# ARPA-SIMC/CRITERIA3D

Measured on AMD Instinct MI355X. Metric: simulated-hours/sec on 512x512x20 grid, higher is better.
Workload: dtype f64

## Files before the change

### criteria3d_amd/csrc/sf3d_control.inc

```

#define SYS_STORE(p, x) __hip_atomic_store((p), (x), __ATOMIC_RELAXED, __HIP_MEMORY_SCOPE_SYSTEM)
#define SYS_LOAD(p) __hip_atomic_load((p), __ATOMIC_RELAXED, __HIP_MEMORY_SCOPE_SYSTEM)

__device__ __forceinline__ unsigned long long rec_lo(double x, uint32_t tag) { return ((unsigned long long)__double_as_longlong(x) & 0xFFFFFFFFull) | ((unsigned long long)tag << 32); }
__device__ __forceinline__ unsigned long long rec_hi(double x, uint32_t tag) { return ((unsigned long long)__double_as_longlong(x) >> 32) | ((unsigned long long)tag << 32); }
__device__ __forceinline__ bool rec_ok(unsigned long long a, unsigned long long b, uint32_t tag) { return (uint32_t)(a >> 32) == tag && (uint32_t)(b >> 32) == tag; }
__device__ __forceinline__ double rec_value(unsigned long long a, unsigned long long b) { return __longlong_as_double((long long)((a & 0xFFFFFFFFull) | (b << 32))); }

__device__ __forceinline__ void dist_combine(double (&acc)[4], const double (&x)[4], int K, int op, bool first)
{
    if (first) { for (int k = 0; k < K; ++k) acc[k] = x[k]; return; }
    if (op == 1) { for (int k = 0; k < K; ++k) acc[k] = dmax(acc[k], x[k]); return; }
    if (op >= 2) {
        dd_merge(acc[0], acc[1], x[0], x[1]);
        if (op == 3) dd_merge(acc[2], acc[3], x[2], x[3]); else for (int k = 2; k < K; ++k) acc[k] += x[k];
        return;
    }
    for (int k = 0; k < K; ++k) acc[k] += x[k];
}
template <int K>
__device__ __forceinline__ bool dist_allgather(const DevView& v, Ctrl* c, double (&vals)[K], int op)
{
    static_assert(K >= 1 && K <= 4, "a mailbox holds four values");
    if (v.world <= 1) return true;
// ... 233 lines not shown
__device__ __forceinline__ void dist_put_node(const DevView& v, uint32_t i, uint32_t par, int field, double val)
{
    const DistView* d = v.dist;
    const uint32_t q = i >> 6, lane = i & 63u;
    for (uint32_t t = d->bndStart[q], t1 = d->bndStart[q + 1]; t < t1; ++t)
        if (d->bndLane[t] == lane) {
            const uint32_t p = d->bndPeer[t];
            SYS_STORE(d->payload[p] + d->sendOff[p] + (size_t)(par * SF3D_DIST_FIELDS + field) * d->sendCount[p] + d->bndSlot[t], val);
        }
}


__device__ __forceinline__ void begin_attempt(Ctrl* c)
{
    c->dt = dmin(c->dtCurr, c->maxTimeStep);
    c->hold = c->cur;
    c->best = -1;
    c->bestMBR = NODATA_D;
    c->approx = 0;
    c->counters[0]++;
    c->stage = ST_APPROX;
}

__global__ void k_step_begin(Ctrl* c, double maxTimeStep)
{
    c->maxTimeStep = maxTimeStep;
    c->seqCount = 0;
    c->aBuf ^= 1u;
    begin_attempt(c);
}

__device__ __forceinline__ void reject_attempt(Ctrl* c)
{
    c->seSource = 2;
    c->cur = c->hold;
    begin_attempt(c);
}

#ifndef SF3D_PROBE_BUDGET
#define SF3D_PROBE_BUDGET 8u
#endif
__device__ __forceinline__ void courant_decision(Ctrl* c, double cmax)
{
    c->counters[2]++;
    c->courant = cmax;
    c->asmSeq++; c->asmSurfOnly = (cmax < 1.01 || c->dt <= c->dtMin) ? 0u : 1u;
    if (cmax < 1.01 || c->dt <= c->dtMin) {
        uint32_t budget = (uint32_t)((c->approx + 1) * ((float)c->maxIter / (float)c->maxApprox));
        c->iterBudget = budget > 25u ? budget : 25u;
        c->iter = 0;
        c->bestNorm = 1.;
// ... 164 lines not shown
```

### criteria3d_amd/csrc/sf3d_device.h

```cpp
#ifndef SF3D_DEVICE_H
#define SF3D_DEVICE_H

#include <stdint.h>

#define SF3D_SLOTS 10
#define SF3D_POOL 5
#define SF3D_BLOCK 256
#define SF3D_CHUNK 64
#define SF3D_MAX_BLOCKS 2048
#define CK_NONE 0
#define CK_MIXED 255

enum : uint8_t { LK_NONE = 0, LK_SOIL_VERT = 1, LK_SOIL_LAT = 2, LK_RUNOFF = 3, LK_INFILTRATION = 4 };

enum : uint32_t {
    ST_IDLE = 0,
    ST_ATTEMPT = 1,
    ST_APPROX = 2,
    ST_SWEEP = 3,
    ST_POST = 4,
    ST_RESTORE = 5,
    ST_ACCEPT = 6,
    ST_DONE = 7,
    ST_FAIL = 8
};

struct alignas(16) sf3d_d2 { double x, y; };
struct alignas(8) sf3d_f2 { float x, y; };

struct SoilDev {
// ... 201 lines not shown
    uint32_t nbSurf, nbSoil;
    double probeMin;
    const uint32_t* chunkList; uint32_t nList, nListSurf;
    const uint32_t* asmList;
    uint32_t pLo, pHi;
    uint32_t aLo, aHi;
    const uint32_t* bndList; uint32_t nBnd;
    const uint16_t* lmask;
    uint32_t haloDirect;
    uint32_t ntStream;
    const DistView* dist;
    int32_t world, rank;
    const uint8_t* owner;
    const ChunkDesc* cdesc;
    const double *z, *size, *pond, *sink;
    const uint16_t* cls;
    const uint8_t* btype;
    const double *bslope, *bsize, *prescribed;
    const uint32_t* lto;
    const uint8_t* lkind;
    const uint8_t* probeMask;
    const double *larea, *ldist;
    double* lflowSum;
    sf3d_d2* A2x[2];
    double *b, *C;
    double* X[SF3D_POOL];
    double *Se, *SeHold, *K, *flow, *bflowRate, *bflowSum;
    double* compatCv; uint8_t* compatCn; double* compatDiag;
    double *cgDiag, *cgR, *cgP, *cgQ;
    double *part0, *part1;
    double *part2, *part3;
    unsigned int* arrive;
    unsigned int* gridBar;
    const SoilDev* soils;
    const double* roughness;
    PairGrid pair;
    ResGrid res;
    Ctrl* ctrl;
    HeatDev heat;
};

struct MapGeo {
    double cohesion;
    double tanFriction;
    double bulkDensity;
    double present;
};
// ... 119 lines not shown
```

### criteria3d_amd/csrc/sf3d_host_build.inc

```

namespace {

template <class F> void parallel_for(uint32_t n, F f)
{
    unsigned nt = std::thread::hardware_concurrency();
    if (nt == 0) nt = 1;
    if (nt > 16) nt = 16;
    if (n < 65536 || nt == 1) { f(0u, n); return; }
    std::vector<std::thread> th;
    const uint32_t chunk = (n + nt - 1) / nt;
    for (unsigned t = 0; t < nt; ++t) {
        const uint32_t a = t * chunk, b = (a + chunk < n) ? a + chunk : n;
        if (a >= b) break;
        th.emplace_back([=] { f(a, b); });
    }
    for (auto& t : th) t.join();
}

const char* kKernelNames[KID_COUNT] = {"k_props", "k_assemble", "k_sweep", "k_post", "k_restore", "k_accept", "k_sweep_pair", "k_sweep_resident", "k_output_map"};

}

sf3d_error_t sf3d_partition_bounds(uint32_t ns, int world, uint32_t* bounds)
{
// ... 92 lines not shown
    }
};

struct SnowCache { float* base = nullptr; uint8_t* mine = nullptr; uint32_t nCells = 0; double lastMs = 0.; bool hourDone = false; };
struct CropCache { float* base = nullptr; CropUnitDev* units = nullptr; uint8_t* mine = nullptr; uint32_t nCells = 0, nUnits = 0; double lastMs[2] = {0., 0.}; };

struct RootCache {
    char* cells = nullptr;
    char* tables = nullptr;
    double* out = nullptr;
    uint8_t* mine = nullptr;
    size_t off[16] = {0};
    uint32_t nCells = 0, nUnits = 0, nSoils = 0, nRows = 0, nrLayers = 0, lunetteMax = 0;
    bool computed = false;
    double lastMs[3] = {0., 0., 0.};
};

struct DeviceSolver::Impl {
    int device = -1;
    hipStream_t stream = nullptr;
    hipStream_t stream2 = nullptr;
    hipEvent_t evLinks[2] = {nullptr, nullptr};
    bool linksPending[2] = {false, false};
    int overlapAccept = -1;
    DevView v{};
    Ctrl* hostCtrl = nullptr;
    std::vector<void*> allocs;
    uint32_t N = 0, ns = 0;
    uint32_t ownedNodes = 0;
    uint32_t lastSweeps = 8;
    uint32_t lastBatches = 1;
    uint32_t predCount = 0, pred[16] = {0};
    uint32_t lastHeatSweeps = 8;
    std::vector<uint32_t> gsLevelStart;
    uint32_t lastHeatSteps = 1;
    double* heatOut[6] = {nullptr};
    double* heatAirP = nullptr;
    std::vector<std::pair<uint32_t, hipGraphExec_t>> graphs;
    int useFused = -1;
    int useGraphs = -1;
    Partition part;
    DistWindow* window = nullptr;
    size_t windowBytes = 0;
    std::vector<void*> peerMaps;
    DistView hostDist{};
    DistView* devDist = nullptr;
// ... 87 lines not shown
             fatal_ = true;                                                                    \
             return SF3D_SOLVER_ERROR; } } while (0)

DeviceSolver& DeviceSolver::instance() { static DeviceSolver s; return s; }
const char* DeviceSolver::kernel_name(int kid) { return (kid >= 0 && kid < KID_COUNT) ? kKernelNames[kid] : nullptr; }

sf3d_error_t DeviceSolver::set_device(int dev)
{
    if (!impl_) impl_ = new Impl();
    int count = 0;
    HIP_TRY(hipGetDeviceCount(&count));
    if (dev < 0 || dev >= count) { snprintf(err_, sizeof(err_), "device %d out of range (%d visible)", dev, count); return SF3D_SOLVER_ERROR; }
    impl_->device = dev;
    HIP_TRY(hipSetDevice(dev));
    return SF3D_OK;
}

static uint64_t g_deviceBytes = 0;
sf3d_error_t DeviceSolver::release()
{
    if (!impl_) return SF3D_OK;
    Impl& I = *impl_;
    if (I.stream) hipStreamSynchronize(I.stream);
    if (I.stream2) hipStreamSynchronize(I.stream2);
    if (I.stream3) hipStreamSynchronize(I.stream3);
#if SF3D_RES_PROFILE
    if (built_ && I.v.res.on && I.v.res.pub) {
        double pr[32];
        if (hipMemcpy(pr, I.v.res.pub, sizeof(pr), hipMemcpyDeviceToHost) == hipSuccess && pr[16] > 0.) {
            const char* names[7] = {"compute + record stores issued", "wave sum + block partial", "halo records", "partial records of all blocks", "barrier B", "norm + decision", "(prologue: per launch, not per iteration)"};
            fprintf(stderr, "[sf3d] resident sweep loop, block 0: %.0f launches, %.2f iterations per launch, %.2f us per launch\n", pr[16], pr[15] / pr[16], pr[17] / pr[16] / 100.);
            for (int p = 0; p < 7; ++p) fprintf(stderr, "[sf3d]   %-40s %7.2f us per iteration\n", names[p], pr[8 + p] / pr[15] / 100.);
        }
    }
#endif
    I.linksPending[0] = I.linksPending[1] = false;
    if (I.stream3) {
        (void)hipStreamDestroy(I.stream3); I.stream3 = nullptr;
        for (auto& ev : I.evSlab) if (ev) { (void)hipEventDestroy(ev); ev = nullptr; }
    }
    I.slabs = -1;
    for (auto& p : I.pending) { I.freeEvents.push_back(p.a); I.freeEvents.push_back(p.b); }
    I.pending.clear();
    for (auto& g : I.graphs) hipGraphExecDestroy(g.second);
    I.graphs.clear();
    for (void* p : I.allocs) hipFree(p);
    I.allocs.clear();
    g_deviceBytes = 0;
    I.maps.free_all();
    if (I.comm && I.pCommDestroy) { I.pCommDestroy(I.comm); I.comm = nullptr; }
    I.rcclMode = false; I.rcclMine = I.rcclGathered = nullptr;
    for (void* p : I.peerMaps) hipIpcCloseMemHandle(p);
    I.peerMaps.clear();
    I.drop_shm();
    if (I.window) { hipFree(I.window); I.window = nullptr; }
    I.devDist = nullptr; I.distStats = nullptr;
    connected_ = false;
    built_ = false;
    fatal_ = false;
    I.overlapAccept = I.useFused = I.useGraphs = I.residentGrids = -1;
    return SF3D_OK;
}

sf3d_error_t DeviceSolver::synchronize()
{
    if (!impl_ || !impl_->stream) return SF3D_OK;
    HIP_TRY(hipStreamSynchronize(impl_->stream));
    if (impl_->stream2) { HIP_TRY(hipStreamSynchronize(impl_->stream2)); impl_->linksPending[0] = impl_->linksPending[1] = false; }
    return SF3D_OK;
}

template <class T> static hipError_t dev_alloc(std::vector<void*>& allocs, T*& p, size_t count)
{
    void* q = nullptr;
    hipError_t e = hipMalloc(&q, (count ? count : 1) * sizeof(T));
    if (e == hipSuccess) { allocs.push_back(q); p = static_cast<T*>(q); g_deviceBytes += (uint64_t)(count ? count : 1) * sizeof(T); }
    return e;
}
uint64_t DeviceSolver::device_bytes() const { return g_deviceBytes; }

static void fill_params(Ctrl& c, const ParamsHost& p)
{
    c.MBRThreshold = p.MBRThreshold; c.residualTolerance = p.residualTolerance;
    c.dtMin = p.dtMin; c.dtMax = p.dtMax; c.lvRatio = p.lvRatio;
    c.courantThreshold = p.courantThreshold; c.instabilityFactor = p.instabilityFactor;
    c.maxApprox = p.maxApprox; c.maxIter = p.maxIter; c.wrc = p.wrc; c.meanType = p.meanType;
    c.dtCurr = p.dtCurr;
    c.lineal = p.lineal ? 1u : 0u;
}

sf3d_error_t DeviceSolver::ensure_device()
// ... 6 lines not shown
        int count = 0;
        HIP_TRY(hipGetDeviceCount(&count));
        if (count <= 0) { snprintf(err_, sizeof(err_), "no HIP device visible: the soilFluxes3D product path has no CPU fallback"); return SF3D_SOLVER_ERROR; }
        if (const char* de = getenv("SF3D_DEVICES")) {
            std::vector<int> list;
            for (const char* q = de; *q;) { char* end = nullptr; const long v = strtol(q, &end, 10); if (end == q) break; list.push_back((int)v); q = (*end == ',') ? end + 1 : end; }
            if (!list.empty()) {
                const int pick = list[(size_t)(dev < 0 ? 0 : dev) % list.size()];
                if (pick < 0 || pick >= count) { snprintf(err_, sizeof(err_), "SF3D_DEVICES names device %d, %d visible", pick, count); return SF3D_SOLVER_ERROR; }
                dev = pick;
            }
        }
        I.device = dev % count;
    }
    HIP_TRY(hipSetDevice(I.device));
    if (!I.stream) HIP_TRY(hipStreamCreateWithFlags(&I.stream, hipStreamNonBlocking));
    return SF3D_OK;
}

sf3d_error_t DeviceSolver::sync_to_device(HostModel& m, const ParamsHost& p)
{
    { const sf3d_error_t e = ensure_device(); if (e != SF3D_OK) return e; }
    Impl& I = *impl_;
    if ((I.linksPending[0] || I.linksPending[1]) && (m.graphDirty || m.stateDirty || m.flowSumsDirty || !built_)) { HIP_TRY(hipStreamSynchronize(I.stream2)); I.linksPending[0] = I.linksPending[1] = false; }
    if (!I.hostCtrl) HIP_TRY(hipHostMalloc((void**)&I.hostCtrl, sizeof(Ctrl), hipHostMallocDefault));

    const uint32_t N = m.N, ns = m.ns;
    const size_t NS = (size_t)N * SF3D_SLOTS;

    if (m.graphDirty || !built_) {
        if (world_ > 1 && connected_) { snprintf(err_, sizeof(err_), "topology changed after sf3d_dist_connect: call sf3d_dist_prepare / export / connect again"); return SF3D_TOPOGRAPHY_ERROR; }
        if (m.surf.size() < N || m.hasClass.size() < N) { snprintf(err_, sizeof(err_), "the model's build arrays were released (a trimmed strip): re-initialise before changing the topology"); return SF3D_TOPOGRAPHY_ERROR; }
        for (uint32_t i = 0; i < N; ++i) {
            if ((m.surf[i] != 0) != (i < ns)) { snprintf(err_, sizeof(err_), "node %u: surface nodes must be exactly the first nrSurfaceNodes indices", i); return SF3D_TOPOGRAPHY_ERROR; }
            if (!m.hasClass[i]) { snprintf(err_, sizeof(err_), "node %u has no soil/surface class", i); return SF3D_MISSING_DATA_ERROR; }
        }
        if (built_) { if (m.hostStaleState) fetch_state(m); if (m.hostStaleFlows) fetch_flows(m); if (m.heat && m.hostStaleHeat && I.v.heat.on) fetch_heat(m); }
        release();
        I.N = N; I.ns = ns;
        DevView& v = I.v;
        v = DevView{};
        v.N = N; v.ns = ns; v.Nnorm = m.globalN ? m.globalN : N;
        v.nChunks = (N + SF3D_CHUNK - 1) / SF3D_CHUNK;
        v.qSplit = (ns + SF3D_CHUNK - 1) / SF3D_CHUNK;
        if (v.qSplit > v.nChunks) v.qSplit = v.nChunks;

        std::vector<uint8_t> kind(NS, LK_NONE);
// ... 360 lines not shown
                            const size_t e = (size_t)sl * N + i;
                            if (kind[e] != LK_NONE && to[e] / SF3D_CHUNK > far) far = to[e] / SF3D_CHUNK;
                        }
                    I.propsNeed[q] = far + 1;
                }
            });
            for (uint32_t q = 1; q < nChunks; ++q) if (I.propsNeed[q] < I.propsNeed[q - 1]) I.propsNeed[q] = I.propsNeed[q - 1];
        }
        {
            const uint32_t per = SF3D_BLOCK / SF3D_CHUNK;
            auto blocks = [&](uint32_t chunks) { uint32_t b = (chunks + per - 1) / per; if (b > SF3D_MAX_BLOCKS) b = SF3D_MAX_BLOCKS; return b; };
            v.nbSoil = blocks(v.nList - v.nListSurf);
            if (const char* be = getenv("SF3D_ASM_SOIL_BLOCKS")) { const uint32_t nb = (uint32_t)atoi(be); if (nb > 0 && nb < v.nbSoil) v.nbSoil = nb; }
        }
        double *z, *size, *pond, *sink, *bslope, *bsize, *prescribed, *roughness, *larea, *ldist;
        uint16_t* cls; uint8_t *btype, *lkind; uint32_t* lto; SoilDev* soils; ChunkDesc* dcdesc;
        HIP_TRY(dev_alloc(I.allocs, z, N)); HIP_TRY(dev_alloc(I.allocs, size, N));
        HIP_TRY(dev_alloc(I.allocs, pond, N)); HIP_TRY(dev_alloc(I.allocs, sink, N));
        HIP_TRY(dev_alloc(I.allocs, cls, N)); HIP_TRY(dev_alloc(I.allocs, btype, N));
        HIP_TRY(dev_alloc(I.allocs, bslope, N)); HIP_TRY(dev_alloc(I.allocs, bsize, N));
        HIP_TRY(dev_alloc(I.allocs, prescribed, N));
        HIP_TRY(dev_alloc(I.allocs, lto, NS)); HIP_TRY(dev_alloc(I.allocs, lkind, NS));
        HIP_TRY(dev_alloc(I.allocs, larea, NS)); HIP_TRY(dev_alloc(I.allocs, ldist, NS));
        HIP_TRY(dev_alloc(I.allocs, v.lflowSum, NS)); HIP_TRY(dev_alloc(I.allocs, v.A2x[0], NS / 2)); HIP_TRY(dev_alloc(I.allocs, v.A2x[1], NS / 2));
        HIP_TRY(dev_alloc(I.allocs, v.b, N)); HIP_TRY(dev_alloc(I.allocs, v.C, N));
        for (int k = 0; k < SF3D_POOL; ++k) HIP_TRY(dev_alloc(I.allocs, v.X[k], N));
        HIP_TRY(dev_alloc(I.allocs, v.Se, N)); HIP_TRY(dev_alloc(I.allocs, v.K, N)); HIP_TRY(dev_alloc(I.allocs, v.SeHold, N));
        HIP_TRY(dev_alloc(I.allocs, dcdesc, (size_t)nChunks));
        uint32_t* dlist; HIP_TRY(dev_alloc(I.allocs, dlist, listSurf.size()));
        if (!listSurf.empty()) HIP_TRY(hipMemcpy(dlist, listSurf.data(), listSurf.size() * 4, hipMemcpyHostToDevice));
        v.chunkList = dlist;
        v.asmList = dlist;
        v.owner = nullptr; v.dist = nullptr;
        {
            const char* e = getenv("SF3D_NT_STREAM");
            const double sweepBytes = 152.0 * (double)v.nList * SF3D_CHUNK;
            v.ntStream = e ? (e[0] != '0') : (sweepBytes > 256.0 * 1024 * 1024);
        }
        {
            v.probeMin = 0.8;
            if (const char* ce = getenv("SF3D_COURANT_PROBE")) { v.probeMin = atof(ce); if (ce[0] == '0' && ce[1] == 0) v.probeMin = -1.; if (ce[0] == 'a') v.probeMin = 0.; }
        }
        I.pairBlocks = 0; I.pairMasked = false; v.pair.masked = 0;
        uint32_t pairOwnLo = 0, pairOwnHi = pairNY;
        if (!pairNode.empty() && world_ > 1) {
            bool ok = true;
            std::vector<int8_t> rowMine(pairNY, -1);
// ... 653 lines not shown
```

### criteria3d_amd/csrc/sf3d_host_step.inc

```
sf3d_error_t DeviceSolver::fetch_state(HostModel& m)
{
    Impl& I = *impl_;
    HIP_TRY(hipMemcpyAsync(m.H.data(), I.v.X[mirror_.cur], (size_t)m.N * 8, hipMemcpyDeviceToHost, I.stream));
    HIP_TRY(hipMemcpyAsync(m.Se.data(), I.v.Se, (size_t)m.N * 8, hipMemcpyDeviceToHost, I.stream));
    HIP_TRY(hipMemcpyAsync(m.K.data(), I.v.K, (size_t)m.N * 8, hipMemcpyDeviceToHost, I.stream));
    HIP_TRY(hipStreamSynchronize(I.stream));
    m.hostStaleState = false;
    return SF3D_OK;
}

sf3d_error_t DeviceSolver::fetch_flows(HostModel& m)
{
    Impl& I = *impl_;
    const size_t N = m.N;
    if (I.stream2) { HIP_TRY(hipStreamSynchronize(I.stream2)); I.linksPending[0] = I.linksPending[1] = false; }
    HIP_TRY(hipMemcpyAsync(m.bflowSum.data(), I.v.bflowSum, N * 8, hipMemcpyDeviceToHost, I.stream));
    HIP_TRY(hipMemcpyAsync(m.bflowRate.data(), I.v.bflowRate, N * 8, hipMemcpyDeviceToHost, I.stream));
    if (I.dslot.empty()) {
        for (int s = 0; s < SF3D_SLOTS; ++s)
            HIP_TRY(hipMemcpyAsync(m.lflowSum[s].data(), I.v.lflowSum + (size_t)s * N, N * 8, hipMemcpyDeviceToHost, I.stream));
        HIP_TRY(hipStreamSynchronize(I.stream));
    } else {
        I.stage.resize(N * SF3D_SLOTS);
        HIP_TRY(hipMemcpyAsync(I.stage.data(), I.v.lflowSum, N * SF3D_SLOTS * 8, hipMemcpyDeviceToHost, I.stream));
        HIP_TRY(hipStreamSynchronize(I.stream));
        for (int s = 0; s < SF3D_SLOTS; ++s) {
            const uint8_t* d = I.dslot.data() + (size_t)s * N; double* dst = m.lflowSum[s].data();
            for (size_t i = 0; i < N; ++i) dst[i] = I.stage[(size_t)d[i] * N + i];
        }
    }
    m.hostStaleFlows = false;
    return SF3D_OK;
}

sf3d_error_t DeviceSolver::fetch_heat(HostModel& m)
{
    Impl& I = *impl_;
    const size_t N = m.N;
// ... 647 lines not shown
            if (I.residentGrids == 0) nbk = SF3D_MAX_BLOCKS;
            I.residentBlocks.push_back({fn, nbk});
        }
        return dim3(v.nb < nbk ? v.nb : nbk);
    };
    if (heatOn && multi) I.useFused = 1;
    const bool fused = !multi && I.useFused;
    const bool fusedMulti = multi && I.useFused;
    const bool linealOn = p.lineal && v.cgDiag != nullptr && !multi && I.useFused;
    const bool resOn = v.res.on && I.resBlocks != 0 && (fused || (fusedMulti && v.haloDirect && !I.rcclMode)) && !linealOn;
    if (resOn && !multi) {
        static const long failAt = getenv("SF3D_RESIDENT_FAIL_TEST") ? strtol(getenv("SF3D_RESIDENT_FAIL_TEST"), nullptr, 10) : -1;
        I.v.res.forceTimeout = (failAt >= 0 && (long)I.stepSeqAll == failAt) ? 1u : 0u;
        ++I.stepSeqAll;
    }
    const bool pairOn = !resOn && (fused || (fusedMulti && v.haloDirect && v.nBnd != 0)) && I.pairBlocks != 0 && !linealOn;
    const dim3 pgrid(I.pushBlocks ? I.pushBlocks : 1);
    hipStream_t st = I.stream;

    const bool timedStep = I.timing == 1 || (I.timing == 2 && (I.stepSeq++ % 8 == 0));
    if (I.overlapAccept < 0) { const char* oe = getenv("SF3D_OVERLAP_ACCEPT"); I.overlapAccept = (oe && oe[0] == '0') ? 0 : 1; }
    if (I.overlapAccept && !multi && !I.stream2) { HIP_TRY(hipStreamCreateWithFlags(&I.stream2, hipStreamNonBlocking)); HIP_TRY(hipEventCreateWithFlags(&I.evLinks[0], hipEventDisableTiming)); HIP_TRY(hipEventCreateWithFlags(&I.evLinks[1], hipEventDisableTiming)); }
    const bool overlap = I.overlapAccept && !multi && I.stream2 && !timedStep && I.timing != 1 && v.compatCv == nullptr;
    auto timed = [&](int kid, auto launch) {
        if (!timedStep || (I.timing == 2 && kid != KID_SWEEP && kid != KID_SWEEP_PAIR && kid != KID_SWEEP_RES)) { launch(); return; }
        hipEvent_t a, b;
        if (I.freeEvents.size() >= 2) { a = I.freeEvents.back(); I.freeEvents.pop_back(); b = I.freeEvents.back(); I.freeEvents.pop_back(); }
        else { hipEventCreate(&a); hipEventCreate(&b); }
        hipEventRecord(a, st); launch(); hipEventRecord(b, st);
        I.pending.push_back({a, b, kid});
    };

    if (heatOn) {
        if (v.heat.save == 2) hipLaunchKernelGGL(k_heat_reset_water_fluxes, grid, block, 0, st, v);
        hipLaunchKernelGGL(k_heat_conductance, grid, block, 0, st, v);
        for (int t = 0; t < SF3D_FLUX_TYPES; ++t) m.lfluxValid[t] = false;
    }
    uint32_t stage = ST_ACCEPT;
    if (m.water) {
    {
        const uint32_t wb = (mirror_.aBuf ^ 1u) & 1u;
        if (I.linksPending[wb]) { HIP_TRY(hipStreamWaitEvent(st, I.evLinks[wb], 0)); I.linksPending[wb] = false; }
        if (!overlap && I.linksPending[wb ^ 1u]) { HIP_TRY(hipStreamWaitEvent(st, I.evLinks[wb ^ 1u], 0)); I.linksPending[wb ^ 1u] = false; }
    }
    {
    hipLaunchKernelGGL(k_step_begin, one, one, 0, st, v.ctrl, maxTimeStep);
    stage = ST_APPROX;
    uint64_t before[8], atStart[8];
    std::memcpy(before, mirror_.counters, sizeof(before));
    std::memcpy(atStart, mirror_.counters, sizeof(atStart));
    int guard = 0;
    uint64_t pairBefore = mirror_.pairLaunches, singleBefore = mirror_.singleLaunches, earlyBefore = mirror_.earlyCourant, resBefore = mirror_.residentLaunches;


    const dim3 propsGrid = resident((const void*)k_props<0, false>), propsHeatGrid = resident((const void*)k_props<0, true>);
    const dim3 acceptGrid = v.ntStream ? resident((const void*)k_accept<true>) : resident((const void*)k_accept<false>);
    auto enqueue_props = [&] {
            if (heatOn && multi) {
                timed(KID_PROPS, [&] { hipLaunchKernelGGL((k_props<2, true>), grid, block, 0, st, v); });
                hipLaunchKernelGGL(k_halo_copy<0>, pgrid, block, 0, st, v);
                hipLaunchKernelGGL(k_heat_halo_water, pgrid, block, 0, st, v);
            }
            else if (heatOn) timed(KID_PROPS, [&] { hipLaunchKernelGGL((k_props<0, true>), propsHeatGrid, block, 0, st, v); });
            else if (multi && fusedMulti) { timed(KID_PROPS, [&] { hipLaunchKernelGGL((k_props<2, false>), grid, block, 0, st, v); }); hipLaunchKernelGGL(k_halo_copy<0>, pgrid, block, 0, st, v); }
            else timed(KID_PROPS, [&] { hipLaunchKernelGGL((k_props<0, false>), propsGrid, block, 0, st, v); });
            if (multi && !fusedMulti) {
                hipLaunchKernelGGL(k_push_kf, pgrid, block, 0, st, v);
                if (I.rcclMode) I.rccl_halo(st, 2);
                hipLaunchKernelGGL(k_sync_kf, one, block, 0, st, v);
// ... 247 lines not shown
            }
            I.pending.clear();
            for (int k = 0; k < KID_COUNT; ++k) {
                std::sort(el[k].begin(), el[k].end(), [](float x, float y) { return x > y; });
                for (size_t q = 0; q < el[k].size() && q < ran[k]; ++q) { I.ms[k] += el[k][q]; I.launches[k]++; }
            }
        }
        std::memcpy(before, c.counters, sizeof(before));
        pairBefore = c.pairLaunches; singleBefore = c.singleLaunches; earlyBefore = c.earlyCourant; resBefore = c.residentLaunches;

        stage = c.stage;
        if (stage != ST_SWEEP && c.iter > 0) I.lastSweeps = c.iter;
        if (stage == ST_ACCEPT || stage == ST_FAIL) break;
        if (++guard > 1000000) { snprintf(err_, sizeof(err_), "step state machine did not terminate (stage %u)", stage); return SF3D_SOLVER_ERROR; }
    }
    {
        const uint64_t used = I.hostCtrl->counters[2] - atStart[2];
        I.lastBatches = used < 1 ? 1u : (uint32_t)used;
        I.predCount = I.hostCtrl->seqCount < 16u ? I.hostCtrl->seqCount : 16u;
        for (uint32_t k = 0; k < I.predCount; ++k) I.pred[k] = I.hostCtrl->seqSweeps[k];
    }
    }
    if (overlap && stage == ST_ACCEPT) {
        uint32_t lcap = 384u; if (const char* le = getenv("SF3D_LINKS_BLOCKS")) lcap = (uint32_t)atoi(le);
        const dim3 lgrid(v.nb > lcap ? lcap : v.nb);
        const Ctrl& hc = *I.hostCtrl;
        const uint32_t rb = hc.acceptABuf & 1u;
        if (v.ntStream) hipLaunchKernelGGL(k_accept_links<true>, lgrid, block, 0, I.stream2, v, hc.acceptBuf, rb, hc.acceptDt);
        else hipLaunchKernelGGL(k_accept_links<false>, lgrid, block, 0, I.stream2, v, hc.acceptBuf, rb, hc.acceptDt);
        HIP_TRY(hipEventRecord(I.evLinks[rb], I.stream2));
        I.linksPending[rb] = true;
    }
    }

    if (heatOn && stage == ST_ACCEPT) {
        hipLaunchKernelGGL(k_heat_begin, one, one, 0, st, v.ctrl, maxTimeStep, m.water ? 1 : 0);
        const dim3 gSaveWater = v.ntStream ? resident((const void*)k_heat_save_water<true>) : resident((const void*)k_heat_save_water<false>), gBoundary = resident((const void*)k_heat_boundary),
                   gHProps = resident((const void*)k_heat_props), gHAsm = v.ntStream ? resident((const void*)k_heat_assemble<true>) : resident((const void*)k_heat_assemble<false>),
                   gHPost = resident((const void*)k_heat_post), gHSave = resident((const void*)k_heat_save);
        hipLaunchKernelGGL(k_heat_save_water_props, resident((const void*)k_heat_save_water_props), block, 0, st, v);
        if (v.ntStream) hipLaunchKernelGGL(k_heat_save_water<true>, gSaveWater, block, 0, st, v); else hipLaunchKernelGGL(k_heat_save_water<false>, gSaveWater, block, 0, st, v);
        int hguard = 0;
        uint32_t lookH = I.lastHeatSteps < 1 ? 1 : (I.lastHeatSteps > 8 ? 8 : I.lastHeatSteps);
        if (v.heat.gs) lookH = 1;
        if (I.useGraphs < 0) { const char* e = getenv("SF3D_GRAPHS"); I.useGraphs = (e && e[0] == '0') ? 0 : 1; }
        auto enqueue_heat = [&](uint32_t steps, uint32_t chunk) {
            for (uint32_t bq = 0; bq < steps; ++bq) {
                hipLaunchKernelGGL(k_heat_boundary, gBoundary, block, 0, st, v);
                hipLaunchKernelGGL(k_heat_props, gHProps, block, 0, st, v);
                if (v.ntStream) hipLaunchKernelGGL(k_heat_assemble<true>, gHAsm, block, 0, st, v); else hipLaunchKernelGGL(k_heat_assemble<false>, gHAsm, block, 0, st, v);
                if (v.heat.gs) {
                    for (uint32_t k = 0; k < chunk; ++k) {
// ... 86 lines not shown
```

### criteria3d_amd/csrc/sf3d_maps.inc

```

#define MAP_GRAVITY 9.80665
#define MAP_NODATA (-9999.0)
enum : int32_t {
    MV_VWC = 0, MV_TOTAL_POTENTIAL = 1, MV_MATRIC_POTENTIAL = 2, MV_AVAILABLE_WATER = 3, MV_DEGREE_OF_SATURATION = 4, MV_AVG_DEGREE_OF_SATURATION = 5,
    MV_WATER_DEFICIT = 9, MV_WATER_INFLOW = 10, MV_WATER_OUTFLOW = 11, MV_FACTOR_OF_SAFETY = 12, MV_MINIMUM_FACTOR_OF_SAFETY = 13,
    MV_SURFACE_POND = 14, MV_MIN_VWC = 15, MV_MAX_VWC = 16
};

__device__ __forceinline__ double map_theta(const SoilDev& s, double Se) { return (Se * (s.thetaS - s.thetaR)) + s.thetaR; }
__device__ __forceinline__ double map_theta_at(const SoilDev& s, double absPsi, uint32_t wrc) { return map_theta(s, se_from_psi(s, absPsi, wrc)); }

__device__ __forceinline__ double map_node_value(const MapView& m, int32_t var, uint32_t i)
{
    const bool surf = i < m.ns;
    switch (var) {
        case MV_VWC: return surf ? (m.H[i] - m.z[i]) : map_theta(m.soils[m.cls[i]], m.Se[i]);
        case MV_TOTAL_POTENTIAL: return m.H[i];
        case MV_MATRIC_POTENTIAL: return m.H[i] - m.z[i];
        case MV_AVAILABLE_WATER: {
            if (surf) return m.H[i] - m.z[i];
            const SoilDev& s = m.soils[m.cls[i]];
            return dmax(0., map_theta(s, m.Se[i]) - map_theta_at(s, 160., m.wrc));
        }
        case MV_DEGREE_OF_SATURATION: {
// ... 132 lines not shown
    if (C.colVer != in.colVer) {
        HIP_TRY(maps_reserve(C.col, C.colCap, colN));
        HIP_TRY(maps_reserve(C.thick, C.thickCap, in.nLayers));
        HIP_TRY(hipMemcpyAsync(C.col, in.col, colN * 4, hipMemcpyHostToDevice, I.stream));
        HIP_TRY(hipMemcpyAsync(C.thick, in.thick, (size_t)in.nLayers * 8, hipMemcpyHostToDevice, I.stream));
        C.colVer = in.colVer;
    }
    if (in.slope && C.slopeVer != in.slopeVer) {
        HIP_TRY(maps_reserve(C.slope, C.slopeCap, 2 * cells));
        HIP_TRY(hipMemcpyAsync(C.slope, in.slope, 2 * cells * 8, hipMemcpyHostToDevice, I.stream));
        C.slopeVer = in.slopeVer;
    }
    if (C.geoHost.size() != in.nGeo || (in.nGeo && std::memcmp(C.geoHost.data(), in.geo, in.nGeo * sizeof(MapGeo)) != 0)) {
        C.geoHost.assign(in.geo, in.geo + in.nGeo);
        HIP_TRY(maps_reserve(C.geo, C.geoCap, in.nGeo));
        HIP_TRY(hipMemcpyAsync(C.geo, C.geoHost.data(), in.nGeo * sizeof(MapGeo), hipMemcpyHostToDevice, I.stream));
    }
    const bool whole = var == MV_MINIMUM_FACTOR_OF_SAFETY || var == MV_AVG_DEGREE_OF_SATURATION;
    const uint32_t lay0 = whole ? 0u : (layer < 0 ? 0u : (uint32_t)layer), lay1 = whole ? 1u : (layer < 0 ? in.nLayers : (uint32_t)layer + 1);
    const size_t outN = (size_t)(lay1 - lay0) * cells;
    HIP_TRY(maps_reserve(C.out, C.outCap, outN));
    if (!C.missing) HIP_TRY(hipMalloc((void**)&C.missing, sizeof(int)));
    HIP_TRY(hipMemsetAsync(C.missing, 0, sizeof(int), I.stream));
    if ((var == MV_WATER_INFLOW || var == MV_WATER_OUTFLOW) && I.stream2) HIP_TRY(hipStreamSynchronize(I.stream2));

    MapView mv{};
    mv.col = C.col; mv.thick = C.thick; mv.slope = C.slope; mv.geo = C.geo;
    mv.H = I.v.X[mirror_.cur]; mv.Se = I.v.Se; mv.z = I.v.z; mv.pond = I.v.pond; mv.lflowSum = I.v.lflowSum;
    mv.cls = I.v.cls; mv.soils = I.v.soils;
    mv.N = I.v.N; mv.ns = I.v.ns; mv.nCells = in.nCells; mv.nLayers = in.nLayers; mv.lay0 = lay0; mv.lay1 = lay1; mv.wrc = p.wrc;
    mv.var = var; mv.flag = flag; mv.out = C.out; mv.missing = C.missing;
    const dim3 grid((in.nCells + SF3D_BLOCK - 1) / SF3D_BLOCK);
    hipEvent_t ev[2] = {nullptr, nullptr};
    if (I.timing) { HIP_TRY(hipEventCreate(&ev[0])); HIP_TRY(hipEventCreate(&ev[1])); HIP_TRY(hipEventRecord(ev[0], I.stream)); }
    if (in.nCells) hipLaunchKernelGGL(k_output_map, grid, dim3(SF3D_BLOCK), 0, I.stream, mv);
    HIP_TRY(hipGetLastError());
    if (I.timing) HIP_TRY(hipEventRecord(ev[1], I.stream));
    HIP_TRY(hipMemcpyAsync(out, C.out, outN * sizeof(float), hipMemcpyDeviceToHost, I.stream));
    int miss = 0;
    HIP_TRY(hipMemcpyAsync(&miss, C.missing, sizeof(int), hipMemcpyDeviceToHost, I.stream));
    HIP_TRY(hipStreamSynchronize(I.stream));
    if (I.timing) {
        float ms = 0.f;
        HIP_TRY(hipEventElapsedTime(&ms, ev[0], ev[1]));
        (void)hipEventDestroy(ev[0]); (void)hipEventDestroy(ev[1]);
        I.launches[KID_MAPS] += 1; I.ms[KID_MAPS] += ms;
    }
// ... 4 lines not shown
```

### criteria3d_amd/csrc/sf3d_phases.inc

```

#define FOR_EACH_CHUNK_OF(list, l0, l1)                                                           \
    const uint32_t lane_ = threadIdx.x & 63u;                                                     \
    const uint32_t wavesTotal_ = gridDim.x * (SF3D_BLOCK / 64);                                   \
    for (uint32_t li_ = __builtin_amdgcn_readfirstlane((l0) + blockIdx.x * (SF3D_BLOCK / 64) + (threadIdx.x >> 6)); \
         li_ < (l1); li_ += wavesTotal_)                                                          \
        for (uint32_t q = __builtin_amdgcn_readfirstlane((list)[li_]), once_ = 1; once_; once_ = 0)
#define FOR_EACH_CHUNK_IN(v, l0, l1) FOR_EACH_CHUNK_OF((v).chunkList, l0, l1)
#define FOR_EACH_CHUNK(v) FOR_EACH_CHUNK_IN(v, 0u, (v).nList)
#define NOT_MINE(v, i) ((i) >= (v).N || ((v).owner != nullptr && (v).owner[i] != (v).rank))

#include "sf3d_heat.inc"

template <bool HEAT>
__device__ __forceinline__ double boundary_update(const DevView& v, const Ctrl* c, uint32_t i, double H, double Ho,
                                                  double z, double K, double Se)
{
    const double dt = c->dt;
    double flow = v.sink[i];
    if (i < v.ns && flow < 0) {
        const double avgH = 0.5 * (H + Ho);
        const double hs = dmax(0., avgH - z);
        const double maxFlux = -hs * v.size[i] / dt;
        flow = dmax(flow, maxFlux);
    }
// ... 837 lines not shown
        accept_links_row<NT>(v, A2, q, i, X, dt);
        if (v.btype[i] != SF3D_BND_NONE) v.bflowSum[i] += v.bflowRate[i] * dt;
    }
}
template <bool NT>
__global__ void __launch_bounds__(SF3D_BLOCK) k_accept(DevView v)
{
    if (v.ctrl->stage != ST_ACCEPT) return;
    body_accept<NT>(v);
}


__global__ void __launch_bounds__(SF3D_BLOCK) k_accept_boundary(DevView v)
{
    const Ctrl* c = v.ctrl;
    if (c->stage != ST_ACCEPT) return;
    const double dt = c->dt;
    FOR_EACH_CHUNK(v) {
        const uint32_t i = q * SF3D_CHUNK + lane_;
        if (NOT_MINE(v, i)) continue;
        if (v.btype[i] != SF3D_BND_NONE) v.bflowSum[i] += v.bflowRate[i] * dt;
    }
}
template <bool NT>
__global__ void __launch_bounds__(SF3D_BLOCK) k_accept_links(DevView v, int xbuf, uint32_t abuf, double dt)
{
    const double* __restrict__ X = v.X[xbuf];
    const sf3d_d2* __restrict__ A2 = v.A2x[abuf & 1u];
    FOR_EACH_CHUNK(v) {
        const uint32_t i = q * SF3D_CHUNK + lane_;
        if (NOT_MINE(v, i)) continue;
        accept_links_row<NT>(v, A2, q, i, X, dt);
    }
}

__global__ void __launch_bounds__(SF3D_BLOCK) k_storage(DevView v)
{
    const Ctrl* c = v.ctrl;
    const double* __restrict__ Xc = v.X[c->cur];
    double st = 0.;
    FOR_EACH_CHUNK(v) {
        const uint32_t i = q * SF3D_CHUNK + lane_;
        if (NOT_MINE(v, i)) continue;
        const double H = Xc[i], z = v.z[i];
        double theta;
        if (i >= v.ns) { const SoilDev s = v.soils[v.cls[i]]; theta = (v.Se[i] * (s.thetaS - s.thetaR)) + s.thetaR; }
        else theta = dmax(H - z, 0.0);
        st += theta * v.size[i];
    }
    const double a = block_sum(st);
    if (threadIdx.x == 0) v.part0[blockIdx.x] = a;
}
```

### criteria3d_amd/csrc/sf3d_physics.inc

```

typedef double sf3d_v2 __attribute__((ext_vector_type(2)));
template <bool NT> __device__ __forceinline__ sf3d_d2 load_coeff(const sf3d_d2* p)
{
    sf3d_v2 t;
    if (NT) t = __builtin_nontemporal_load(reinterpret_cast<const sf3d_v2*>(p));
    else t = *reinterpret_cast<const sf3d_v2*>(p);
    sf3d_d2 r; r.x = t.x; r.y = t.y; return r;
}
template <bool NT> __device__ __forceinline__ void store_coeff(sf3d_d2* p, double x, double y)
{
    sf3d_v2 t; t.x = x; t.y = y;
    if (NT) __builtin_nontemporal_store(t, reinterpret_cast<sf3d_v2*>(p));
    else *reinterpret_cast<sf3d_v2*>(p) = t;
}
typedef float sf3d_fv2 __attribute__((ext_vector_type(2)));
template <bool NT> __device__ __forceinline__ sf3d_f2 load_f2(const sf3d_f2* p)
{
    sf3d_fv2 t;
    if (NT) t = __builtin_nontemporal_load(reinterpret_cast<const sf3d_fv2*>(p));
    else t = *reinterpret_cast<const sf3d_fv2*>(p);
    sf3d_f2 r; r.x = t.x; r.y = t.y; return r;
}
template <bool NT> __device__ __forceinline__ void store_f2(sf3d_f2* p, float x, float y)
{
// ... 82 lines not shown
    return exp(x);
#endif
}
extern "C" __device__ double __ocml_powr_f64(double, double);
__device__ __forceinline__ double ppow(double x, double y)
{
#if SF3D_FAST_POW
    return sf3d_fpow(x, y);
#else
    return __ocml_powr_f64(x, y);
#endif
}
__device__ __forceinline__ double pcbrt(double x)
{
#if SF3D_FAST_POW
    return sf3d_fcbrt(x);
#else
    return cbrt(x);
#endif
}
__device__ __forceinline__ double tortuosity(double Se, double L) { return (L == 0.5) ? sqrt(Se) : ppow(Se, L); }
#endif

__device__ __forceinline__ sf3d_d2* cur_A2(const DevView& v) { return v.A2x[v.ctrl->aBuf & 1u]; }

__device__ __forceinline__ int free_buffer3(int cur, int hold, int best)
{
    for (int b = 0; b < SF3D_POOL; ++b)
        if (b != cur && b != hold && b != best) return b;
    return 0;
}
__device__ __forceinline__ int free_buffer(const Ctrl* c) { return free_buffer3(c->cur, c->hold, c->best); }

__device__ __forceinline__ void free_buffers2(const Ctrl* c, int& f1, int& f2)
{
    uint32_t used = (1u << c->cur) | (1u << c->hold);
    if (c->best >= 0) used |= 1u << c->best;
    uint32_t fr = ~used & ((1u << SF3D_POOL) - 1u);
    f1 = __builtin_ctz(fr); fr &= fr - 1u;
    f2 = __builtin_ctz(fr);
}

__device__ __forceinline__ double block_sum(double v)
{
    __shared__ double sm[SF3D_BLOCK / 64];
    for (int off = 32; off > 0; off >>= 1) v += __shfl_down(v, off, 64);
    const int lane = threadIdx.x & 63, wave = threadIdx.x >> 6;
// ... 137 lines not shown
```

Measured before the change: 43.87.

## Batch deferred accept-links updates across several steps with multi-buffered coefficients

Adds an optional queue that defers the k_accept_links flux accumulation over up to SF3D_LINKS_DEFER accepted steps. Each deferred step keeps its own coefficient buffer and a head snapshot. A single batched kernel then reads and writes lflowSum once for the whole batch instead of once per step. The default depth is 1, so without the env var every step launches immediately, as before, but through the new batched kernel and the new buffer-rotation logic. Deeper batching adds memory and device-to-device snapshot copies in exchange for less lflowSum traffic.

```diff
diff --git a/criteria3d_amd/csrc/sf3d_control.inc b/criteria3d_amd/csrc/sf3d_control.inc
--- a/criteria3d_amd/csrc/sf3d_control.inc
+++ b/criteria3d_amd/csrc/sf3d_control.inc
@@ -279,11 +279,11 @@
     c->stage = ST_APPROX;
 }
 
-__global__ void k_step_begin(Ctrl* c, double maxTimeStep)
+__global__ void k_step_begin(Ctrl* c, double maxTimeStep, uint32_t nA2)
 {
     c->maxTimeStep = maxTimeStep;
     c->seqCount = 0;
-    c->aBuf ^= 1u;
+    if (c->acceptABuf == c->aBuf) c->aBuf = (c->aBuf + 1u) % nA2;
     begin_attempt(c);
 }
 
diff --git a/criteria3d_amd/csrc/sf3d_device.h b/criteria3d_amd/csrc/sf3d_device.h
--- a/criteria3d_amd/csrc/sf3d_device.h
+++ b/criteria3d_amd/csrc/sf3d_device.h
@@ -6,6 +6,7 @@
 #define SF3D_SLOTS 10
 #define SF3D_POOL 5
 #define SF3D_BLOCK 256
+#define SF3D_LINKS_MAX 8
 #define SF3D_CHUNK 64
 #define SF3D_MAX_BLOCKS 2048
 #define CK_NONE 0
@@ -253,7 +254,8 @@
     const uint8_t* probeMask;
     const double *larea, *ldist;
     double* lflowSum;
-    sf3d_d2* A2x[2];
+    sf3d_d2* A2x[SF3D_LINKS_MAX + 1];
+    uint32_t nA2;
     double *b, *C;
     double* X[SF3D_POOL];
     double *Se, *SeHold, *K, *flow, *bflowRate, *bflowSum;
diff --git a/criteria3d_amd/csrc/sf3d_host_build.inc b/criteria3d_amd/csrc/sf3d_host_build.inc
--- a/criteria3d_amd/csrc/sf3d_host_build.inc
+++ b/criteria3d_amd/csrc/sf3d_host_build.inc
@@ -138,6 +138,29 @@
     hipStream_t stream2 = nullptr;
     hipEvent_t evLinks[2] = {nullptr, nullptr};
     bool linksPending[2] = {false, false};
+    uint32_t acceptSeq = 0;
+    int linksDepth = -1;
+    double* headSnap[SF3D_LINKS_MAX] = {nullptr};
+    LinkBatch linkQueue{};
+    uint32_t linksCap = 0;
+    hipError_t launch_links()
+    {
+        if (linkQueue.n == 0) return hipSuccess;
+        const dim3 lgrid(v.nb > linksCap ? linksCap : v.nb);
+        if (v.ntStream) hipLaunchKernelGGL(k_accept_links<true>, lgrid, dim3(SF3D_BLOCK), 0, stream2, v, linkQueue);
+        else hipLaunchKernelGGL(k_accept_links<false>, lgrid, dim3(SF3D_BLOCK), 0, stream2, v, linkQueue);
+        linkQueue.n = 0;
+        return hipGetLastError();
+    }
+    hipError_t flush_links()
+    {
+        if (!stream2) return hipSuccess;
+        hipError_t e = launch_links();
+        if (e != hipSuccess) return e;
+        e = hipStreamSynchronize(stream2);
+        linksPending[0] = linksPending[1] = false;
+        return e;
+    }
     int overlapAccept = -1;
     DevView v{};
     Ctrl* hostCtrl = nullptr;
@@ -271,6 +294,9 @@
     if (!impl_) return SF3D_OK;
     Impl& I = *impl_;
     if (I.stream) hipStreamSynchronize(I.stream);
+    if (built_) (void)I.flush_links();
+    I.linkQueue.n = 0; I.linksDepth = -1;
+    for (auto& hs : I.headSnap) hs = nullptr;
     if (I.stream2) hipStreamSynchronize(I.stream2);
     if (I.stream3) hipStreamSynchronize(I.stream3);
 #if SF3D_RES_PROFILE
@@ -283,7 +309,6 @@
         }
     }
 #endif
-    I.linksPending[0] = I.linksPending[1] = false;
     if (I.stream3) {
         (void)hipStreamDestroy(I.stream3); I.stream3 = nullptr;
         for (auto& ev : I.evSlab) if (ev) { (void)hipEventDestroy(ev); ev = nullptr; }
@@ -315,7 +340,7 @@
 {
     if (!impl_ || !impl_->stream) return SF3D_OK;
     HIP_TRY(hipStreamSynchronize(impl_->stream));
-    if (impl_->stream2) { HIP_TRY(hipStreamSynchronize(impl_->stream2)); impl_->linksPending[0] = impl_->linksPending[1] = false; }
+    HIP_TRY(impl_->flush_links());
     return SF3D_OK;
 }
 
@@ -368,7 +393,7 @@
 {
     { const sf3d_error_t e = ensure_device(); if (e != SF3D_OK) return e; }
     Impl& I = *impl_;
-    if ((I.linksPending[0] || I.linksPending[1]) && (m.graphDirty || m.stateDirty || m.flowSumsDirty || !built_)) { HIP_TRY(hipStreamSynchronize(I.stream2)); I.linksPending[0] = I.linksPending[1] = false; }
+    if ((I.linksPending[0] || I.linksPending[1] || I.linkQueue.n) && (m.graphDirty || m.stateDirty || m.flowSumsDirty || !built_)) HIP_TRY(I.flush_links());
     if (!I.hostCtrl) HIP_TRY(hipHostMalloc((void**)&I.hostCtrl, sizeof(Ctrl), hipHostMallocDefault));
 
     const uint32_t N = m.N, ns = m.ns;
@@ -775,7 +800,7 @@
         HIP_TRY(dev_alloc(I.allocs, prescribed, N));
         HIP_TRY(dev_alloc(I.allocs, lto, NS)); HIP_TRY(dev_alloc(I.allocs, lkind, NS));
         HIP_TRY(dev_alloc(I.allocs, larea, NS)); HIP_TRY(dev_alloc(I.allocs, ldist, NS));
-        HIP_TRY(dev_alloc(I.allocs, v.lflowSum, NS)); HIP_TRY(dev_alloc(I.allocs, v.A2x[0], NS / 2)); HIP_TRY(dev_alloc(I.allocs, v.A2x[1], NS / 2));
+        HIP_TRY(dev_alloc(I.allocs, v.lflowSum, NS)); HIP_TRY(dev_alloc(I.allocs, v.A2x[0], NS / 2)); HIP_TRY(dev_alloc(I.allocs, v.A2x[1], NS / 2)); v.nA2 = 2;
         HIP_TRY(dev_alloc(I.allocs, v.b, N)); HIP_TRY(dev_alloc(I.allocs, v.C, N));
         for (int k = 0; k < SF3D_POOL; ++k) HIP_TRY(dev_alloc(I.allocs, v.X[k], N));
         HIP_TRY(dev_alloc(I.allocs, v.Se, N)); HIP_TRY(dev_alloc(I.allocs, v.K, N)); HIP_TRY(dev_alloc(I.allocs, v.SeHold, N));
diff --git a/criteria3d_amd/csrc/sf3d_host_step.inc b/criteria3d_amd/csrc/sf3d_host_step.inc
--- a/criteria3d_amd/csrc/sf3d_host_step.inc
+++ b/criteria3d_amd/csrc/sf3d_host_step.inc
@@ -13,7 +13,7 @@
 {
     Impl& I = *impl_;
     const size_t N = m.N;
-    if (I.stream2) { HIP_TRY(hipStreamSynchronize(I.stream2)); I.linksPending[0] = I.linksPending[1] = false; }
+    HIP_TRY(I.flush_links());
     HIP_TRY(hipMemcpyAsync(m.bflowSum.data(), I.v.bflowSum, N * 8, hipMemcpyDeviceToHost, I.stream));
     HIP_TRY(hipMemcpyAsync(m.bflowRate.data(), I.v.bflowRate, N * 8, hipMemcpyDeviceToHost, I.stream));
     if (I.dslot.empty()) {
@@ -707,6 +707,35 @@
     if (I.overlapAccept < 0) { const char* oe = getenv("SF3D_OVERLAP_ACCEPT"); I.overlapAccept = (oe && oe[0] == '0') ? 0 : 1; }
     if (I.overlapAccept && !multi && !I.stream2) { HIP_TRY(hipStreamCreateWithFlags(&I.stream2, hipStreamNonBlocking)); HIP_TRY(hipEventCreateWithFlags(&I.evLinks[0], hipEventDisableTiming)); HIP_TRY(hipEventCreateWithFlags(&I.evLinks[1], hipEventDisableTiming)); }
     const bool overlap = I.overlapAccept && !multi && I.stream2 && !timedStep && I.timing != 1 && v.compatCv == nullptr;
+    if (I.linksDepth < 0) {
+        int D = 1;
+        if (const char* de = getenv("SF3D_LINKS_DEFER")) D = atoi(de);
+        if (D > SF3D_LINKS_MAX) D = SF3D_LINKS_MAX;
+        if (D < 1 || !I.overlapAccept || multi || !I.stream2 || v.compatCv != nullptr) D = 1;
+        I.linksCap = 384u;
+        if (const char* le = getenv("SF3D_LINKS_BLOCKS")) I.linksCap = (uint32_t)atoi(le);
+        if (I.linksCap == 0) I.linksCap = 1;
+        if (D > 1) {
+            const size_t NS2 = (size_t)v.N * SF3D_SLOTS / 2;
+            std::vector<void*> got;
+            bool ok = true;
+            for (int k = 0; k < 2 * (D - 1) && ok; ++k) {
+                void* q = nullptr;
+                if (hipMalloc(&q, k < D - 1 ? NS2 * sizeof(sf3d_d2) : (size_t)v.N * 8) == hipSuccess) got.push_back(q); else ok = false;
+            }
+            if (!ok) { (void)hipGetLastError(); for (void* q : got) (void)hipFree(q); D = 1; }
+            else {
+                for (int k = 0; k < D - 1; ++k) {
+                    I.v.A2x[2 + k] = static_cast<sf3d_d2*>(got[k]); I.headSnap[k] = static_cast<double*>(got[D - 1 + k]);
+                    HIP_TRY(hipMemsetAsync(v.A2x[2 + k], 0, NS2 * sizeof(sf3d_d2), st));
+                    g_deviceBytes += NS2 * sizeof(sf3d_d2) + (uint64_t)v.N * 8;
+                }
+                for (void* q : got) I.allocs.push_back(q);
+                I.v.nA2 = (uint32_t)D + 1;
+            }
+        }
+        I.linksDepth = D;
+    }
     auto timed = [&](int kid, auto launch) {
         if (!timedStep || (I.timing == 2 && kid != KID_SWEEP && kid != KID_SWEEP_PAIR && kid != KID_SWEEP_RES)) { launch(); return; }
         hipEvent_t a, b;
@@ -724,12 +753,13 @@
     uint32_t stage = ST_ACCEPT;
     if (m.water) {
     {
-        const uint32_t wb = (mirror_.aBuf ^ 1u) & 1u;
-        if (I.linksPending[wb]) { HIP_TRY(hipStreamWaitEvent(st, I.evLinks[wb], 0)); I.linksPending[wb] = false; }
-        if (!overlap && I.linksPending[wb ^ 1u]) { HIP_TRY(hipStreamWaitEvent(st, I.evLinks[wb ^ 1u], 0)); I.linksPending[wb ^ 1u] = false; }
+        const uint32_t ob = I.acceptSeq & 1u;
+        if (!overlap && I.linkQueue.n) { HIP_TRY(I.launch_links()); HIP_TRY(hipEventRecord(I.evLinks[ob ^ 1u], I.stream2)); I.linksPending[ob ^ 1u] = true; }
+        if (I.linksPending[ob]) { HIP_TRY(hipStreamWaitEvent(st, I.evLinks[ob], 0)); I.linksPending[ob] = false; }
+        if (!overlap && I.linksPending[ob ^ 1u]) { HIP_TRY(hipStreamWaitEvent(st, I.evLinks[ob ^ 1u], 0)); I.linksPending[ob ^ 1u] = false; }
     }
     {
-    hipLaunchKernelGGL(k_step_begin, one, one, 0, st, v.ctrl, maxTimeStep);
+    hipLaunchKernelGGL(k_step_begin, one, one, 0, st, v.ctrl, maxTimeStep, v.nA2);
     stage = ST_APPROX;
     uint64_t before[8], atStart[8];
     std::memcpy(before, mirror_.counters, sizeof(before));
@@ -1023,12 +1053,16 @@
     }
     }
     if (overlap && stage == ST_ACCEPT) {
-        uint32_t lcap = 384u; if (const char* le = getenv("SF3D_LINKS_BLOCKS")) lcap = (uint32_t)atoi(le);
-        const dim3 lgrid(v.nb > lcap ? lcap : v.nb);
         const Ctrl& hc = *I.hostCtrl;
-        const uint32_t rb = hc.acceptABuf & 1u;
-        if (v.ntStream) hipLaunchKernelGGL(k_accept_links<true>, lgrid, block, 0, I.stream2, v, hc.acceptBuf, rb, hc.acceptDt);
-        else hipLaunchKernelGGL(k_accept_links<false>, lgrid, block, 0, I.stream2, v, hc.acceptBuf, rb, hc.acceptDt);
+        LinkBatch& lq = I.linkQueue;
+        const uint32_t k = lq.n++;
+        lq.A2[k] = v.A2x[hc.acceptABuf]; lq.dt[k] = hc.acceptDt; lq.X[k] = v.X[hc.acceptBuf];
+        if (lq.n >= (uint32_t)I.linksDepth) HIP_TRY(I.launch_links());
+        else {
+            HIP_TRY(hipMemcpyAsync(I.headSnap[k], v.X[hc.acceptBuf], (size_t)v.N * 8, hipMemcpyDeviceToDevice, I.stream2));
+            lq.X[k] = I.headSnap[k];
+        }
+        const uint32_t rb = I.acceptSeq++ & 1u;
         HIP_TRY(hipEventRecord(I.evLinks[rb], I.stream2));
         I.linksPending[rb] = true;
     }
diff --git a/criteria3d_amd/csrc/sf3d_maps.inc b/criteria3d_amd/csrc/sf3d_maps.inc
--- a/criteria3d_amd/csrc/sf3d_maps.inc
+++ b/criteria3d_amd/csrc/sf3d_maps.inc
@@ -178,7 +178,7 @@
     HIP_TRY(maps_reserve(C.out, C.outCap, outN));
     if (!C.missing) HIP_TRY(hipMalloc((void**)&C.missing, sizeof(int)));
     HIP_TRY(hipMemsetAsync(C.missing, 0, sizeof(int), I.stream));
-    if ((var == MV_WATER_INFLOW || var == MV_WATER_OUTFLOW) && I.stream2) HIP_TRY(hipStreamSynchronize(I.stream2));
+    if (var == MV_WATER_INFLOW || var == MV_WATER_OUTFLOW) HIP_TRY(I.flush_links());
 
     MapView mv{};
     mv.col = C.col; mv.thick = C.thick; mv.slope = C.slope; mv.geo = C.geo;
diff --git a/criteria3d_amd/csrc/sf3d_phases.inc b/criteria3d_amd/csrc/sf3d_phases.inc
--- a/criteria3d_amd/csrc/sf3d_phases.inc
+++ b/criteria3d_amd/csrc/sf3d_phases.inc
@@ -883,15 +883,66 @@
         if (v.btype[i] != SF3D_BND_NONE) v.bflowSum[i] += v.bflowRate[i] * dt;
     }
 }
+struct LinkBatch {
+    uint32_t n, pad;
+    const double* X[SF3D_LINKS_MAX];
+    const sf3d_d2* A2[SF3D_LINKS_MAX];
+    double dt[SF3D_LINKS_MAX];
+};
 template <bool NT>
-__global__ void __launch_bounds__(SF3D_BLOCK) k_accept_links(DevView v, int xbuf, uint32_t abuf, double dt)
-{
-    const double* __restrict__ X = v.X[xbuf];
-    const sf3d_d2* __restrict__ A2 = v.A2x[abuf & 1u];
+__global__ void __launch_bounds__(SF3D_BLOCK) k_accept_links(DevView v, LinkBatch lb)
+{
+    const uint32_t n = lb.n;
     FOR_EACH_CHUNK(v) {
         const uint32_t i = q * SF3D_CHUNK + lane_;
         if (NOT_MINE(v, i)) continue;
-        accept_links_row<NT>(v, A2, q, i, X, dt);
+        double a[SF3D_SLOTS], xj[SF3D_SLOTS], f[SF3D_SLOTS], Hi;
+        uint32_t j[SF3D_SLOTS];
+        const ChunkDesc cd = v.cdesc[q];
+        #pragma unroll
+        for (int s = 0; s < SF3D_SLOTS; ++s) {
+            if (cd.kind[s] != CK_MIXED) j[s] = i + cd.delta[s];
+            else if ((cd.sweepUniform >> s) & 1u) { const uint32_t jj = i + (uint32_t)cd.delta[s]; j[s] = jj < v.N ? jj : i; }
+            else j[s] = v.lto[(size_t)s * v.N + i];
+        }
+        {   const sf3d_d2* __restrict__ A2 = lb.A2[0]; const double* __restrict__ X = lb.X[0];
+            #pragma unroll
+            for (int p = 0; p < SF3D_SLOTS / 2; ++p) { const sf3d_d2 t = load_coeff<NT>(&A2[(size_t)p * v.N + i]); a[2 * p] = t.x; a[2 * p + 1] = t.y; }
+            Hi = X[i];
+            #pragma unroll
+            for (int s = 0; s < SF3D_SLOTS; ++s) xj[s] = X[j[s]];
+        }
+        uint32_t have = 0;
+        #pragma unroll
+        for (int s = 0; s < SF3D_SLOTS; ++s) { const bool on = a[s] != 0.; f[s] = on ? load_stream<NT>(&v.lflowSum[(size_t)s * v.N + i]) : 0.; have |= on ? 1u << s : 0u; }
+        #pragma unroll 1
+        for (uint32_t k = 0; k < n; ++k) {
+            double an[SF3D_SLOTS], xn[SF3D_SLOTS], Hn = 0.;
+            if (k + 1 < n) {
+                const sf3d_d2* __restrict__ A2 = lb.A2[k + 1]; const double* __restrict__ X = lb.X[k + 1];
+                #pragma unroll
+                for (int p = 0; p < SF3D_SLOTS / 2; ++p) { const sf3d_d2 t = load_coeff<NT>(&A2[(size_t)p * v.N + i]); an[2 * p] = t.x; an[2 * p + 1] = t.y; }
+                Hn = X[i];
+                #pragma unroll
+                for (int s = 0; s < SF3D_SLOTS; ++s) xn[s] = X[j[s]];
+            } else {
+                #pragma unroll
+                for (int s = 0; s < SF3D_SLOTS; ++s) { an[s] = 0.; xn[s] = 0.; }
+            }
+            const double dt = lb.dt[k];
+            #pragma unroll
+            for (int s = 0; s < SF3D_SLOTS; ++s)
+                if (a[s] != 0.) {
+                    if (!((have >> s) & 1u)) { f[s] = load_stream<NT>(&v.lflowSum[(size_t)s * v.N + i]); have |= 1u << s; }
+                    f[s] = f[s] + a[s] * (Hi - xj[s]) * dt;
+                }
+            #pragma unroll
+            for (int s = 0; s < SF3D_SLOTS; ++s) { a[s] = an[s]; xj[s] = xn[s]; }
+            Hi = Hn;
+        }
+        #pragma unroll
+        for (int s = 0; s < SF3D_SLOTS; ++s)
+            if ((have >> s) & 1u) store_stream<NT>(&v.lflowSum[(size_t)s * v.N + i], f[s]);
     }
 }
 
diff --git a/criteria3d_amd/csrc/sf3d_physics.inc b/criteria3d_amd/csrc/sf3d_physics.inc
--- a/criteria3d_amd/csrc/sf3d_physics.inc
+++ b/criteria3d_amd/csrc/sf3d_physics.inc
@@ -128,7 +128,7 @@
 __device__ __forceinline__ double tortuosity(double Se, double L) { return (L == 0.5) ? sqrt(Se) : ppow(Se, L); }
 #endif
 
-__device__ __forceinline__ sf3d_d2* cur_A2(const DevView& v) { return v.A2x[v.ctrl->aBuf & 1u]; }
+__device__ __forceinline__ sf3d_d2* cur_A2(const DevView& v) { return v.A2x[v.ctrl->aBuf]; }
 
 __device__ __forceinline__ int free_buffer3(int cur, int hold, int best)
 {
```

After: 42.93. 0.979x the previous value.
